# FanmingL/Recurrent-Offpolicy-RL

Hardware: AMD Instinct MI355X
Metric: env-steps/sec trained (higher is better)
Workload: dtype f32; 1 GPU; smamba_s32_c16_b2_nln SAC-REDQ update, B=64/GPU, T=1024, D=256 (configs[1]; N=8: configs[3]); row_length=1043, obs=17, act=6, critic=efc-8, global_rows=64, parallelism=dp1

## Files before the change

recurrent-offpolicy-rl_amd/csrc/gemm_bf3.hip:

```cpp
#include "gemm_splitk.h"
#include "gemm_call.h"

namespace {
using namespace resel;

typedef float f32x16 __attribute__((ext_vector_type(16)));
typedef __bf16 bf16x8 __attribute__((ext_vector_type(8)));
constexpr int BM = 256, BN = 128;
constexpr int NTH = 512;
constexpr int GRID = 256;
constexpr int TILE = BM * BN;
constexpr int ROWB = 64;
constexpr int PLA = BM * ROWB, PLB = BN * ROWB;
constexpr int STAGE = 3 * PLA + 3 * PLB;

struct Params {
    const float *A, *B, *bias;
    float *C, *slab;
    int64_t lda, ldb, ldc, sA, sB, sC, sBias;
    int M, N, K;
    int act;
    int mt, nt;
    int nfull, nsplit, nsl, kslice;
    const float *amaxA, *amaxB;
    AmaxOut amaxC;
    int ntst;
    const float* aux;
    int64_t ldaux, sAux;
    float* red;
    int redrows;
};

__device__ __forceinline__ int plane_off(int row, int c) {
    const int q = row >> 2;
    return ((row ^ (q & 1)) << 6) + ((c ^ (q & 3)) << 4);
}

__device__ __forceinline__ uint32_t rne_pair(float lo, float hi) {
    typedef __bf16 bf16x2_t __attribute__((ext_vector_type(2)));
    typedef float f32x2_t __attribute__((ext_vector_type(2)));
    const f32x2_t v = {lo, hi};
    return __builtin_bit_cast(uint32_t, __builtin_convertvector(v, bf16x2_t));
}
struct P3 { uint2 p1, p2, p3; };
template <int NP>
__device__ __forceinline__ P3 split4(const float4& v) {
#ifdef BF3_AB_NOSPLIT
    return P3{make_uint2(__float_as_uint(v.x), __float_as_uint(v.y)), make_uint2(__float_as_uint(v.z), __float_as_uint(v.w)),
              make_uint2(__float_as_uint(v.x), __float_as_uint(v.w))};
#endif
    const float x[4] = {v.x, v.y, v.z, v.w};
    uint32_t w1[2], w2[2], w3[2] = {0u, 0u};
#pragma unroll
    for (int q = 0; q < 2; ++q) {
        const uint32_t u0 = __float_as_uint(x[2 * q]), u1 = __float_as_uint(x[2 * q + 1]);
        w1[q] = __builtin_amdgcn_perm(u1, u0, 0x07060302u);
        const float r0 = x[2 * q] - __uint_as_float(u0 & 0xffff0000u), r1 = x[2 * q + 1] - __uint_as_float(u1 & 0xffff0000u);
        if (NP == 2) {
            w2[q] = rne_pair(r0, r1);
        } else {
            const uint32_t v0 = __float_as_uint(r0), v1 = __float_as_uint(r1);
            w2[q] = __builtin_amdgcn_perm(v1, v0, 0x07060302u);
            const float s0 = r0 - __uint_as_float(v0 & 0xffff0000u), s1 = r1 - __uint_as_float(v1 & 0xffff0000u);
            w3[q] = __builtin_amdgcn_perm(__float_as_uint(s1), __float_as_uint(s0), 0x07060302u);
        }
    }
    return P3{make_uint2(w1[0], w1[1]), make_uint2(w2[0], w2[1]), make_uint2(w3[0], w3[1])};
}
struct P3h { uint32_t p1, p2, p3; };
template <int NP>
__device__ __forceinline__ P3h split2(float x0, float x1) {
    const uint32_t u0 = __float_as_uint(x0), u1 = __float_as_uint(x1);
    P3h o;
    o.p1 = __builtin_amdgcn_perm(u1, u0, 0x07060302u);
    const float r0 = x0 - __uint_as_float(u0 & 0xffff0000u), r1 = x1 - __uint_as_float(u1 & 0xffff0000u);
    if (NP == 2) {
        o.p2 = rne_pair(r0, r1);
        o.p3 = 0u;
        return o;
    }
    const uint32_t v0 = __float_as_uint(r0), v1 = __float_as_uint(r1);
    o.p2 = __builtin_amdgcn_perm(v1, v0, 0x07060302u);
    const float s0 = r0 - __uint_as_float(v0 & 0xffff0000u), s1 = r1 - __uint_as_float(v1 & 0xffff0000u);
    o.p3 = __builtin_amdgcn_perm(__float_as_uint(s1), __float_as_uint(s0), 0x07060302u);
    return o;
}

typedef _Float16 f16x2_t __attribute__((ext_vector_type(2)));
typedef float f32x2_t __attribute__((ext_vector_type(2)));
template <bool WIDE>
__device__ __forceinline__ void split_pair_f16(float x0, float x1, f32x2_t sc, uint32_t& p1, uint32_t& p2, uint32_t& p3) {
#ifdef BF3_AB_NOSPLIT
    p1 = __float_as_uint(x0); p2 = __float_as_uint(x1); p3 = __float_as_uint(x0) ^ __float_as_uint(sc.x);
    return;
#endif
    const f32x2_t xs = {x0 * sc.x, x1 * sc.x};
    const f16x2_t h = __builtin_convertvector(xs, f16x2_t);
    p1 = __builtin_bit_cast(uint32_t, h);
    if (WIDE) {
        const f32x2_t r = {__builtin_fmaf((float)h.x, -2048.f, x0 * sc.y), __builtin_fmaf((float)h.y, -2048.f, x1 * sc.y)};
        p2 = __builtin_bit_cast(uint32_t, __builtin_convertvector(r, f16x2_t));
        p3 = 0u;
    } else {
        const f32x2_t r = {xs.x - (float)h.x, xs.y - (float)h.y};
        p2 = __builtin_bit_cast(uint32_t, __builtin_convertvector(r, f16x2_t));
        p3 = 0u;
    }
}
template <bool WIDE>
__device__ __forceinline__ P3 split4_f16(const float4& v, f32x2_t sc) {
    P3 o;
    split_pair_f16<WIDE>(v.x, v.y, sc, o.p1.x, o.p2.x, o.p3.x);
    split_pair_f16<WIDE>(v.z, v.w, sc, o.p1.y, o.p2.y, o.p3.y);
// ... 379 lines not shown
            }
            BF3_FENCE();
            cur_st ^= 1;
        }
        if (F16) {
#pragma unroll
            for (int a = 0; a < 2; ++a)
#pragma unroll
                for (int b = 0; b < 2; ++b)
#pragma unroll
                    for (int e = 0; e < 16; ++e) acc[a][b][e] *= unscale;
        }
#ifdef BF3_AB_NOEPI
        if (lane == 0) p.C[(int64_t)cur.m0 * p.ldc + cur.n0 + w] = acc[0][0][0] + acc[0][1][1] + acc[1][0][2] + acc[1][1][3];
        continue;
#endif
        if (cur.split) {
            slab_store<BN>(p.slab + (int64_t)(cur.split - 1) * TILE + (wm + 4 * lh) * BN + wn + li, acc);
        } else {
            float* C = p.C + (int64_t)cur.z * p.sC;
            const bool full_m = cur.m0 + BM <= p.M;
#pragma unroll
            for (int b = 0; b < 2; ++b) {
                const int n = cur.n0 + wn + 32 * b + li;
                if (n >= p.N) continue;
#pragma unroll
                for (int a = 0; a < 2; ++a) {
                    float v[16];
#pragma unroll
                    for (int e = 0; e < 16; ++e) v[e] = acc[a][b][e] + bv[b];
                    if (p.act == 1) {
#pragma unroll
                        for (int e = 0; e < 16; ++e) v[e] = elu1(v[e]);
                    }
                    if (p.act == 3) {
#pragma unroll
                        for (int e = 0; e < 16; ++e) v[e] = softplus_nb(v[e]);
                    }
                    const int mb = cur.m0 + wm + 32 * a + 4 * lh;
                    float* crow = C + (int64_t)mb * p.ldc + n;
                    if (p.act == 2) {
#pragma unroll
                        for (int e = 0; e < 16; ++e) {
                            const int dm = (e & 3) + 8 * (e >> 2);
                            if (mb + dm < p.M) v[e] += crow[(int64_t)dm * p.ldc];
                        }
                    }
                    if (full_m) {
#pragma unroll
                        for (int e = 0; e < 16; ++e) crow[(int64_t)((e & 3) + 8 * (e >> 2)) * p.ldc] = v[e];
                    } else {
#pragma unroll
                        for (int e = 0; e < 16; ++e) {
                            const int dm = (e & 3) + 8 * (e >> 2);
                            if (mb + dm < p.M) crow[(int64_t)dm * p.ldc] = v[e];
                        }
                    }
                    if (p.amaxC.slot) {
#pragma unroll
                        for (int e = 0; e < 16; e += 2) cmax = fmaxf(cmax, fmaxf(__builtin_fabsf(v[e]), __builtin_fabsf(v[e + 1])));
                    }
                }
            }
        }
    }
    amax_publish_wave(cmax, p.amaxC);
#ifdef BF3_AB_CLOCK
    if (tid == 0) {
        g_bf3_clock[2 * blockIdx.x] = __builtin_amdgcn_s_memtime() - ck_t0;
        g_bf3_clock[2 * blockIdx.x + 1] = __builtin_amdgcn_s_memrealtime() - ck_r0;
    }
#endif
}

constexpr int NTH_WS = 512;
constexpr int WS_LDS = 2 * STAGE;
#define WS_BARRIER() asm volatile("s_waitcnt lgkmcnt(0)\n\ts_barrier" ::: "memory")

template <bool AKC, bool BKC, int EPI = 0>
__global__ __launch_bounds__(NTH_WS, 1) void gemm_ws_kernel(Params p) {
    static_assert(EPI == 0 || EPI == 4 || EPI == 5, "EPI: 0 plain, 4 dact, 5 head (the act codes of the fused host entries)");
    extern __shared__ __attribute__((aligned(16))) char lds[];
    const int tid = threadIdx.x;
    const int total = p.nfull + p.nsplit * p.nsl;
    const int G = gridDim.x;
    if ((int)blockIdx.x >= total) return;
    const float sa_ = f16_scale(amax_read(p.amaxA)), sb_ = f16_scale(amax_read(p.amaxB));
    asm volatile("" :: "v"(sa_), "v"(sb_));

    if (__builtin_amdgcn_readfirstlane(tid) >= 256) {
        const int pt = tid - 256;
        const f32x2_t scA = {sa_, 2048.f * sa_}, scB = {sb_, 2048.f * sb_};
        typedef Src<AKC, BM> SA;
        typedef Src<BKC, BN> SB;
        SA a0, a1;
        SB b0, b1;
        a0.init_lds(pt); a1.init_lds(pt + 256);
        b0.init_lds(pt); b1.init_lds(pt + 256);
        typedef float f32x4a __attribute__((ext_vector_type(4)));
        f32x4a ra[2][2][SA::NR], rb[2][2][SB::NR];
        int nsteps = 0;
        for (int it = blockIdx.x; it < total; it += G) {
            const Item i = decode<BM, BN>(p, it);
            nsteps += (i.kend - i.kbeg + BK - 1) / BK;
        }
        int p_item = blockIdx.x, p_k0 = 0, p_kend = 0;
        bool p_live = true;
        auto p_open = [&]() {
            const Item it = decode<BM, BN>(p, p_item);
            const float* Ab = p.A + (int64_t)it.z * p.sA;
            const float* Bb = p.B + (int64_t)it.z * p.sB;
            a0.init(Ab, p.lda, p.M, it.m0, it.kbeg, pt); a1.init(Ab, p.lda, p.M, it.m0, it.kbeg, pt + 256);
            b0.init(Bb, p.ldb, p.N, it.n0, it.kbeg, pt); b1.init(Bb, p.ldb, p.N, it.n0, it.kbeg, pt + 256);
            p_k0 = it.kbeg; p_kend = it.kend;
        };
        auto advance = [&]() {
            a0.base += a0.step; a1.base += a1.step; b0.base += b0.step; b1.base += b1.step;
            p_k0 += BK;
            if (p_k0 >= p_kend) {
                p_item += G;
                if (p_item < total) p_open(); else p_live = false;
            }
        };
        auto aload = [&](f32x4a& r, const char* base, uint32_t off) {
#ifdef BF3_AB_NOLOAD
            asm volatile("" : "+v"(r) : "v"(off), "s"(base) : "memory");
#else
            asm volatile("global_load_dwordx4 %0, %1, %2" : "=v"(r) : "v"(off), "s"(base) : "memory");
#endif
        };
        auto issue_set = [&](auto SET) {
            constexpr int S = decltype(SET)::value;
            auto all = [&](auto& src, auto& regs) {
                typedef std::remove_reference_t<decltype(src)> ST;
#pragma unroll
                for (int i = 0; i < ST::NR; ++i) {
                    if constexpr (ST::is_kc) aload(regs[i], src.base, src.piece_off(i));
                    else aload(regs[i], src.base, src.off[i]);
                }
            };
            all(a0, ra[S][0]); all(a1, ra[S][1]); all(b0, rb[S][0]); all(b1, rb[S][1]);
            advance();
        };
        auto recycle = [&](auto SET, auto MODEC) {
            constexpr int S = decltype(SET)::value;
            constexpr int MODE = decltype(MODEC)::value;
            constexpr bool LOAD = MODE == 0;
            uint32_t st_off = S * STAGE;
            asm volatile("" : "+s"(st_off));
            char* st = lds + st_off;
            auto one = [&](auto& src, auto& regs, char* pl, f32x2_t sc, auto PLc, auto WIDEc) {
                constexpr int PL = decltype(PLc)::value;
                constexpr bool WIDE = decltype(WIDEc)::value;
                typedef std::remove_reference_t<decltype(src)> ST;
                if constexpr (ST::is_kc) {
#pragma unroll
                    for (int i = 0; i < ST::NR; ++i) {
                        if (LOAD) asm volatile("s_waitcnt vmcnt(23)" : "+v"(regs[i]) :: "memory");
                        const float4 v = make_float4(regs[i].x, regs[i].y, regs[i].z, regs[i].w);
                        const P3 sp = split4_f16<WIDE>(v, sc);
                        char* d = pl + src.loff[0] + 4096 * i;
                        *reinterpret_cast<uint2*>(d) = sp.p1;
                        *reinterpret_cast<uint2*>(d + PL) = sp.p2;
                        if (MODE != 1) aload(regs[i], src.base, src.piece_off(i));
                    }
                } else {
                    float4 t[ST::NR];
                    if constexpr (ST::NR == 4) { if (LOAD) asm volatile("s_waitcnt vmcnt(20)" : "+v"(regs[0]), "+v"(regs[1]), "+v"(regs[2]), "+v"(regs[3]) :: "memory"); }
                    else { if (LOAD) asm volatile("s_waitcnt vmcnt(22)" : "+v"(regs[0]), "+v"(regs[1]) :: "memory"); }
#pragma unroll
                    for (int i = 0; i < ST::NR; ++i) t[i] = make_float4(regs[i].x, regs[i].y, regs[i].z, regs[i].w);
                    src.template store_from<PL, 2, WIDE ? 1 : 2>(t, pl, sc);
                    if (MODE != 1) {
#pragma unroll
                        for (int i = 0; i < ST::NR; ++i) aload(regs[i], src.base, src.off[i]);
                    }
                }
            };
            using IA = std::integral_constant<int, PLA>;
            using IB = std::integral_constant<int, PLB>;
            one(a0, ra[S][0], st, scA, IA{}, std::true_type{});
            one(a1, ra[S][1], st, scA, IA{}, std::true_type{});
            one(b0, rb[S][0], st + 3 * PLA, scB, IB{}, std::false_type{});
            one(b1, rb[S][1], st + 3 * PLA, scB, IB{}, std::false_type{});
            if (MODE != 1) advance();
        };
        auto landed = [&]() {
#pragma unroll
            for (int q = 0; q < 2; ++q)
#pragma unroll
                for (int v = 0; v < 2; ++v) {
#pragma unroll
                    for (int i = 0; i < SA::NR; ++i) asm volatile("s_waitcnt vmcnt(0)" : "+v"(ra[q][v][i]) :: "memory");
#pragma unroll
                    for (int i = 0; i < SB::NR; ++i) asm volatile("s_waitcnt vmcnt(0)" : "+v"(rb[q][v][i]) :: "memory");
                }
        };
        using S0 = std::integral_constant<int, 0>;
        using S1 = std::integral_constant<int, 1>;
        using M0 = std::integral_constant<int, 0>;
        using M1 = std::integral_constant<int, 1>;
        using M2 = std::integral_constant<int, 2>;
        p_open();
        issue_set(S0{});
        if (nsteps > 1) issue_set(S1{});
        int j = 0;
        for (; j + 3 < nsteps; j += 2) {
            recycle(S0{}, M0{});
            WS_BARRIER();
            recycle(S1{}, M0{});
            WS_BARRIER();
        }
        landed();
        for (; j < nsteps; ++j) {
            const bool more = j + 2 < nsteps;
            if (j & 1) { if (more) recycle(S1{}, M2{}); else recycle(S1{}, M1{}); }
            else { if (more) recycle(S0{}, M2{}); else recycle(S0{}, M1{}); }
            if (more) landed();
            WS_BARRIER();
        }
        WS_BARRIER();
        return;
    }

    const float unscale = (1.f / sa_) * (1.f / sb_);
    const int lane = tid & 63, w = tid >> 6;
    const int wm = (w >> 1) * 128, wn = (w & 1) * 64;
    const int li = lane & 31, lh = lane >> 5;
    const char* fa[2];
    const char* fb[2];
#pragma unroll
    for (int s = 0; s < 2; ++s) {
        fa[s] = lds + wm * ROWB + plane_off(li, 2 * s + lh);
        fb[s] = lds + 3 * PLA + wn * ROWB + plane_off(li, 2 * s + lh);
    }
    struct F4 { f16x8 a[2][4], b[2][2]; };
    auto rd = [&](F4& f, const char* pa, const char* pb) {
#pragma unroll
        for (int pi = 0; pi < 2; ++pi) {
#pragma unroll
            for (int t = 0; t < 4; ++t) f.a[pi][t] = *reinterpret_cast<const f16x8*>(pa + pi * PLA + t * 32 * ROWB);
#pragma unroll
            for (int t = 0; t < 2; ++t) f.b[pi][t] = *reinterpret_cast<const f16x8*>(pb + pi * PLB + t * 32 * ROWB);
        }
    };
    f32x16 acc[4][2];
    auto mm = [&](const F4& f) {
        const f16x8 k = {(_Float16)0.00048828125f, (_Float16)0.00048828125f, (_Float16)0.00048828125f, (_Float16)0.00048828125f,
                         (_Float16)0.00048828125f, (_Float16)0.00048828125f, (_Float16)0.00048828125f, (_Float16)0.00048828125f};
        const f16x8 bs0 = f.b[0][0] * k, bs1 = f.b[0][1] * k;
#ifdef BF3_AB_NOMFMA
#pragma unroll
        for (int a = 0; a < 4; ++a) asm volatile("" :: "v"(f.a[0][a]), "v"(f.a[1][a]), "v"(bs0), "v"(bs1), "v"(f.b[0][0]), "v"(f.b[0][1]), "v"(f.b[1][0]), "v"(f.b[1][1]));
        return;
#endif
#pragma unroll
        for (int a = 0; a < 4; ++a) {
            acc[a][0] = __builtin_amdgcn_mfma_f32_32x32x16_f16(f.a[1][a], bs0, acc[a][0], 0, 0, 0);
            acc[a][1] = __builtin_amdgcn_mfma_f32_32x32x16_f16(f.a[1][a], bs1, acc[a][1], 0, 0, 0);
        }
#pragma unroll
        for (int q = 1; q >= 0; --q)
#pragma unroll
            for (int a = 0; a < 4; ++a) {
                acc[a][0] = __builtin_amdgcn_mfma_f32_32x32x16_f16(f.a[0][a], f.b[q][0], acc[a][0], 0, 0, 0);
                acc[a][1] = __builtin_amdgcn_mfma_f32_32x32x16_f16(f.a[0][a], f.b[q][1], acc[a][1], 0, 0, 0);
            }
    };
    float cmax = 0.f;
    F4 f0, f1;
    WS_BARRIER();
    rd(f0, fa[0], fb[0]);
    int cur_st = 0;
    constexpr bool DEFER_F0 = EPI == 4;
    for (int c_item = blockIdx.x; c_item < total; c_item += G) {
        const Item cur = decode<BM, BN>(p, c_item);
        if (DEFER_F0 && c_item != (int)blockIdx.x) rd(f0, fa[0] + cur_st * STAGE, fb[0] + cur_st * STAGE);
        float zero = 0.f;
        asm volatile("" : "+v"(zero));
#pragma unroll
        for (int a = 0; a < 4; ++a)
#pragma unroll
            for (int b = 0; b < 2; ++b)
#pragma unroll
                for (int e = 0; e < 16; ++e) acc[a][b][e] = zero;
        float bv[2] = {0.f, 0.f};
        for (int c_k0 = cur.kbeg; c_k0 < cur.kend; c_k0 += BK) {
            const int so = cur_st * STAGE, sn = (cur_st ^ 1) * STAGE;
            if (c_k0 + BK >= cur.kend && p.bias && !cur.split) {
#pragma unroll
                for (int b = 0; b < 2; ++b) {
                    const int n = cur.n0 + wn + 32 * b + li;
                    bv[b] = p.bias[(int64_t)cur.z * p.sBias + (n < p.N ? n : 0)];
                }
            }
            BF3_FENCE();
            rd(f1, fa[1] + so, fb[1] + so);
            mm(f0);
#pragma unroll
            for (int i = 0; i < 12; ++i) {
                __builtin_amdgcn_sched_group_barrier(0x008, 1, 0);
                __builtin_amdgcn_sched_group_barrier(0x100, 1, 0);
            }
            BF3_FENCE();
            WS_BARRIER();
            BF3_FENCE();
            if (!(DEFER_F0 && c_k0 + BK >= cur.kend)) rd(f0, fa[0] + sn, fb[0] + sn);
            mm(f1);
#pragma unroll
            for (int i = 0; i < 12; ++i) {
                __builtin_amdgcn_sched_group_barrier(0x008, 1, 0);
                __builtin_amdgcn_sched_group_barrier(0x100, 1, 0);
            }
            BF3_FENCE();
            cur_st ^= 1;
        }
#ifdef BF3_AB_NOEPI
        if (lane == 0) p.C[(int64_t)cur.m0 * p.ldc + cur.n0 + w] = acc[0][0][0] + acc[1][1][1] + acc[2][0][2] + acc[3][1][3];
        continue;
#endif
#pragma unroll
        for (int a = 0; a < 4; ++a)
#pragma unroll
            for (int b = 0; b < 2; ++b)
#pragma unroll
                for (int e = 0; e < 16; ++e) acc[a][b][e] *= unscale;
        if (cur.split) {
            float* o = p.slab + (int64_t)(cur.split - 1) * TILE + (wm + 4 * lh) * BN + wn + li;
#pragma unroll
            for (int a = 0; a < 4; ++a)
#pragma unroll
                for (int b = 0; b < 2; ++b)
#pragma unroll
                    for (int e = 0; e < 16; ++e) o[(32 * a + (e & 3) + 8 * (e >> 2)) * BN + 32 * b] = acc[a][b][e];
            continue;
        }
        if constexpr (EPI == 0) {
            float* C = p.C + (int64_t)cur.z * p.sC;
            const bool full_m = cur.m0 + BM <= p.M;
            if (full_m && cur.n0 + BN <= p.N && p.act != 2) {
                char* sc = lds + (w >> 1) * STAGE + 2 * PLA + (w & 1) * 5120;
                float* wr = reinterpret_cast<float*>(sc) + (4 * lh) * 40 + li;
                const float4* rdp = reinterpret_cast<const float4*>(sc + (lane >> 3) * 160 + (lane & 7) * 16);
#pragma unroll
                for (int b = 0; b < 2; ++b) {
#pragma unroll
                    for (int a = 0; a < 4; ++a) {
                        float v[16];
#pragma unroll
                        for (int e = 0; e < 16; ++e) v[e] = acc[a][b][e] + bv[b];
                        if (p.act == 1) {
#pragma unroll
                            for (int e = 0; e < 16; ++e) v[e] = elu1(v[e]);
                        }
                        if (p.act == 3) {
#pragma unroll
                            for (int e = 0; e < 16; ++e) v[e] = softplus_nb(v[e]);
                        }
                        if (p.amaxC.slot) {
#pragma unroll
                            for (int e = 0; e < 16; e += 2) cmax = fmaxf(cmax, fmaxf(__builtin_fabsf(v[e]), __builtin_fabsf(v[e + 1])));
                        }
#pragma unroll
                        for (int e = 0; e < 16; ++e) wr[((e & 3) + 8 * (e >> 2)) * 40] = v[e];
                        float* q = C + (int64_t)(cur.m0 + wm + 32 * a + (lane >> 3)) * p.ldc + cur.n0 + wn + 32 * b + 4 * (lane & 7);
#pragma unroll
                        for (int g = 0; g < 4; ++g) {
                            const float4 t = rdp[g * 8 * 10];
                            if (p.ntst) {
                                typedef float f4v __attribute__((ext_vector_type(4)));
                                __builtin_nontemporal_store(f4v{t.x, t.y, t.z, t.w}, reinterpret_cast<f4v*>(q + (int64_t)(8 * g) * p.ldc));
                            } else {
                                *reinterpret_cast<float4*>(q + (int64_t)(8 * g) * p.ldc) = t;
                            }
                        }
                    }
                }
                continue;
            }
#pragma unroll
            for (int b = 0; b < 2; ++b) {
                const int n = cur.n0 + wn + 32 * b + li;
                if (n >= p.N) continue;
#pragma unroll
                for (int a = 0; a < 4; ++a) {
                    float v[16];
#pragma unroll
                    for (int e = 0; e < 16; ++e) v[e] = acc[a][b][e] + bv[b];
                    if (p.act == 1) {
#pragma unroll
                        for (int e = 0; e < 16; ++e) v[e] = elu1(v[e]);
                    }
                    if (p.act == 3) {
#pragma unroll
                        for (int e = 0; e < 16; ++e) v[e] = softplus_nb(v[e]);
                    }
                    const int mb = cur.m0 + wm + 32 * a + 4 * lh;
                    float* crow = C + (int64_t)mb * p.ldc + n;
                    if (p.act == 2) {
#pragma unroll
                        for (int e = 0; e < 16; ++e) {
                            const int dm = (e & 3) + 8 * (e >> 2);
                            if (mb + dm < p.M) v[e] += crow[(int64_t)dm * p.ldc];
                        }
                    }
                    if (full_m) {
#pragma unroll
                        for (int e = 0; e < 16; ++e) crow[(int64_t)((e & 3) + 8 * (e >> 2)) * p.ldc] = v[e];
                    } else {
#pragma unroll
                        for (int e = 0; e < 16; ++e) {
                            const int dm = (e & 3) + 8 * (e >> 2);
                            if (mb + dm < p.M) crow[(int64_t)dm * p.ldc] = v[e];
                        }
                    }
                    if (p.amaxC.slot) {
#pragma unroll
                        for (int e = 0; e < 16; e += 2) cmax = fmaxf(cmax, fmaxf(__builtin_fabsf(v[e]), __builtin_fabsf(v[e + 1])));
                    }
                }
            }
        } else if constexpr (EPI == 4) {
            float* C = p.C + (int64_t)cur.z * p.sC;
            constexpr int PF = 3;
            const int lane = (int)__builtin_amdgcn_mbcnt_hi(~0u, __builtin_amdgcn_mbcnt_lo(~0u, 0u));
            const int li = lane & 31, lh = lane >> 5;
            const int w = __builtin_amdgcn_readfirstlane(threadIdx.x >> 6);
            const int wm = (w >> 1) * 128, wn = (w & 1) * 64;
            typedef float f32x4a __attribute__((ext_vector_type(4)));
            f32x4a yv[8][4];
            char* sc = lds + (w >> 1) * STAGE + 2 * PLA + (w & 1) * 5120;
            float* wr = reinterpret_cast<float*>(sc) + (4 * lh) * 40 + li;
            float4* rdp = reinterpret_cast<float4*>(sc + (lane >> 3) * 160 + (lane & 7) * 16);
            const uint32_t ylane = (uint32_t)(((lane >> 3) * (int)p.ldaux + 4 * (lane & 7)) * 4);
            const float* ybase = p.aux + (int64_t)cur.z * p.sAux + (int64_t)(cur.m0 + wm) * p.ldaux + cur.n0 + wn;
            auto yld = [](f32x4a& r, uint32_t off, const float* base) {
                asm volatile("global_load_dwordx4 %0, %1, %2" : "=v"(r) : "v"(off), "s"(base) : "memory");
            };
            auto ywait = [](f32x4a& r0, f32x4a& r1, f32x4a& r2, f32x4a& r3, auto NC) {
                asm volatile("s_waitcnt vmcnt(%4)" : "+v"(r0), "+v"(r1), "+v"(r2), "+v"(r3) : "n"(decltype(NC)::value) : "memory");
            };
            auto yload = [&](auto TC) {
                constexpr int t = decltype(TC)::value;
                if constexpr (t < 8) {
                    const float* yb = ybase + (int64_t)(32 * (t >> 1)) * p.ldaux + 32 * (t & 1);
#pragma unroll
                    for (int g = 0; g < 4; ++g) yld(yv[t][g], ylane, yb + (int64_t)(8 * g) * p.ldaux);
                }
            };
            float cs[2] = {0.f, 0.f}, cmx = 0.f;
            auto mul = [&](auto TC) {
                constexpr int t = decltype(TC)::value;
                constexpr int a = t >> 1, b = t & 1;
                yload(std::integral_constant<int, t + PF>{});
                ywait(yv[t][0], yv[t][1], yv[t][2], yv[t][3], std::integral_constant<int, 4 * ((t + PF < 7 ? t + PF : 7) - t)>{});
#pragma unroll
                for (int g = 0; g < 4; ++g) rdp[g * 8 * 10] = make_float4(yv[t][g].x, yv[t][g].y, yv[t][g].z, yv[t][g].w);
#pragma unroll
                for (int e = 0; e < 16; ++e) {
                    const float y = wr[((e & 3) + 8 * (e >> 2)) * 40];
                    const float v = acc[a][b][e] * (y > 0.f ? 1.f : y + 1.f);
                    acc[a][b][e] = v;
                    cs[b] += v;
                    cmx = fmaxf(cmx, __builtin_fabsf(v));
                }
            };
            yload(std::integral_constant<int, 0>{}); yload(std::integral_constant<int, 1>{}); yload(std::integral_constant<int, 2>{});
            static_assert(PF == 3, "the prologue issues PF tiles");
            mul(std::integral_constant<int, 0>{}); mul(std::integral_constant<int, 1>{}); mul(std::integral_constant<int, 2>{});
            mul(std::integral_constant<int, 3>{}); mul(std::integral_constant<int, 4>{}); mul(std::integral_constant<int, 5>{});
            mul(std::integral_constant<int, 6>{}); mul(std::integral_constant<int, 7>{});
            if (p.red) {
#pragma unroll
                for (int b = 0; b < 2; ++b) {
                    const float c = cs[b] + __shfl_xor(cs[b], 32, 64);
                    if (lh == 0) p.red[((int64_t)cur.z * p.redrows + 2 * (cur.m0 / BM) + (w >> 1)) * p.N + cur.n0 + wn + 32 * b + li] = c;
                }
            }
            amax_publish_wave(cmx, p.amaxC);
#pragma unroll
            for (int b = 0; b < 2; ++b) {
#pragma unroll
                for (int a = 0; a < 4; ++a) {
#pragma unroll
                    for (int e = 0; e < 16; ++e) wr[((e & 3) + 8 * (e >> 2)) * 40] = acc[a][b][e];
                    float* q = C + (int64_t)(cur.m0 + wm + 32 * a + (lane >> 3)) * p.ldc + cur.n0 + wn + 32 * b + 4 * (lane & 7);
#pragma unroll
                    for (int g = 0; g < 4; ++g) {
                        const float4 t = rdp[g * 8 * 10];
                        typedef float f4v __attribute__((ext_vector_type(4)));
                        __builtin_nontemporal_store(f4v{t.x, t.y, t.z, t.w}, reinterpret_cast<f4v*>(q + (int64_t)(8 * g) * p.ldc));
                    }
                }
            }
        } else {
            float* C = p.C + (int64_t)cur.z * p.sC;
            const bool full_m = cur.m0 + BM <= p.M;
            if (full_m && cur.n0 + BN <= p.N) {
                char* sc = lds + (w >> 1) * STAGE + 2 * PLA + (w & 1) * 5120;
                float* wr = reinterpret_cast<float*>(sc) + (4 * lh) * 40 + li;
                const float4* rdp = reinterpret_cast<const float4*>(sc + (lane >> 3) * 160 + (lane & 7) * 16);
                auto tile = [&](int a, int b, const float4& w3, float (&qr)[4]) {
                    float v[16];
#pragma unroll
                    for (int e = 0; e < 16; ++e) v[e] = acc[a][b][e] + bv[b];
#pragma unroll
                    for (int e = 0; e < 16; ++e) v[e] = elu1(v[e]);
                    if (p.amaxC.slot) {
#pragma unroll
                        for (int e = 0; e < 16; e += 2) cmax = fmaxf(cmax, fmaxf(__builtin_fabsf(v[e]), __builtin_fabsf(v[e + 1])));
                    }
#pragma unroll
                    for (int e = 0; e < 16; ++e) wr[((e & 3) + 8 * (e >> 2)) * 40] = v[e];
                    float* q = C + (int64_t)(cur.m0 + wm + 32 * a + (lane >> 3)) * p.ldc + cur.n0 + wn + 32 * b + 4 * (lane & 7);
#pragma unroll
                    for (int g = 0; g < 4; ++g) {
                        float4 t = rdp[g * 8 * 10];
                        qr[g] += (t.x * w3.x + t.y * w3.y) + (t.z * w3.z + t.w * w3.w);
                        if (p.ntst) {
                            typedef float f4v __attribute__((ext_vector_type(4)));
                            __builtin_nontemporal_store(f4v{t.x, t.y, t.z, t.w}, reinterpret_cast<f4v*>(q + (int64_t)(8 * g) * p.ldc));
                        } else {
                            *reinterpret_cast<float4*>(q + (int64_t)(8 * g) * p.ldc) = t;
                        }
                    }
                };
                float4 w3[2];
#pragma unroll
                for (int b = 0; b < 2; ++b) w3[b] = ld4(p.aux + (int64_t)cur.z * p.sAux + cur.n0 + wn + 32 * b + 4 * (lane & 7));
#pragma unroll
                for (int a = 0; a < 4; ++a) {
                    float qr[4] = {0.f, 0.f, 0.f, 0.f};
#pragma unroll
                    for (int b = 0; b < 2; ++b) tile(a, b, w3[b], qr);
                    float* qp = p.red + ((int64_t)cur.z * 2 * p.nt + 2 * (cur.n0 / BN) + (w & 1)) * p.M + cur.m0 + wm + 32 * a + (lane >> 3);
#pragma unroll
                    for (int g = 0; g < 4; ++g) {
                        float r = qr[g];
                        r += __shfl_xor(r, 1, 64); r += __shfl_xor(r, 2, 64); r += __shfl_xor(r, 4, 64);
                        if ((lane & 7) == 0) qp[8 * g] = r;
                    }
                }
                continue;
            }
#pragma unroll
            for (int a = 0; a < 4; ++a) {
                float qe[16];
#pragma unroll
                for (int e = 0; e < 16; ++e) qe[e] = 0.f;
                const int mb = cur.m0 + wm + 32 * a + 4 * lh;
#pragma unroll
                for (int b = 0; b < 2; ++b) {
                    const int n = cur.n0 + wn + 32 * b + li;
                    if (n >= p.N) continue;
                    float v[16];
#pragma unroll
                    for (int e = 0; e < 16; ++e) v[e] = acc[a][b][e] + bv[b];
#pragma unroll
                    for (int e = 0; e < 16; ++e) v[e] = elu1(v[e]);
                    const float w3 = p.aux[(int64_t)cur.z * p.sAux + n];
#pragma unroll
                    for (int e = 0; e < 16; ++e) qe[e] += v[e] * w3;
                    float* crow = C + (int64_t)mb * p.ldc + n;
                    if (full_m) {
#pragma unroll
                        for (int e = 0; e < 16; ++e) crow[(int64_t)((e & 3) + 8 * (e >> 2)) * p.ldc] = v[e];
                    } else {
#pragma unroll
                        for (int e = 0; e < 16; ++e) {
                            const int dm = (e & 3) + 8 * (e >> 2);
                            if (mb + dm < p.M) crow[(int64_t)dm * p.ldc] = v[e];
                        }
                    }
                    if (p.amaxC.slot) {
#pragma unroll
                        for (int e = 0; e < 16; e += 2) cmax = fmaxf(cmax, fmaxf(__builtin_fabsf(v[e]), __builtin_fabsf(v[e + 1])));
                    }
                }
                float* qp = p.red + ((int64_t)cur.z * 2 * p.nt + 2 * (cur.n0 / BN) + (w & 1)) * p.M;
#pragma unroll
                for (int e = 0; e < 16; ++e) {
                    float r = qe[e];
#pragma unroll
                    for (int o = 1; o < 32; o <<= 1) r += __shfl_xor(r, o, 64);
                    const int m = mb + (e & 3) + 8 * (e >> 2);
                    if (li == 0 && m < p.M) qp[m] = r;
                }
            }
        }
    }
    amax_publish_wave(cmax, p.amaxC);
}

template <bool AKC, bool BKC, int SP>
int launch_one(const Params& p, dim3 grid, hipStream_t s) {
    static std::atomic<bool> attr_set[64];
    return launch_big_lds(gemm_bf3_kernel<AKC, BKC, SP>, attr_set, grid, dim3(NTH), 2 * STAGE, s, p);
}
template <bool AKC, bool BKC, int EPI = 0>
int launch_ws(const Params& p, dim3 grid, hipStream_t s) {
    static std::atomic<bool> attr_set[64];
    return launch_big_lds(gemm_ws_kernel<AKC, BKC, EPI>, attr_set, grid, dim3(NTH_WS), WS_LDS, s, p);
}

constexpr int g_nt = 1;

}

#ifdef BF3_AB_CLOCK
extern "C" int resel_bf3_debug_clock(unsigned long long* host_out) {
    return (int)hipMemcpyFromSymbol(host_out, HIP_SYMBOL(g_bf3_clock), sizeof(unsigned long long) * 2 * GRID);
}
#endif

namespace resel {

size_t gemm_bf3_workspace_bytes(int M, int N, int K, int batch) {
    const Plan pl = make_plan<BM, BN, GRID>(M, N, K, batch);
    return (size_t)pl.nsplit * pl.nsl * TILE * sizeof(float);
}

inline bool whole_k_steps(int K, int kslice) { return K % BK == 0 && kslice % BK == 0; }

bool gemm_bf3_fused_ok(int M, int N, int K) { return M > 128 && N >= 4 && K >= BK && whole_k_steps(K, K); }

int gemm_bf3_launch(const GemmCall& c, int split, const GemmFused& fused) {
    if (split == 2 && (!c.amax_a || !c.amax_b)) return RESEL_EINVAL;
    const int M = c.M, N = c.N, K = c.K, act = c.act;
    Plan pl = make_plan<BM, BN, GRID>(M, N, K, c.batch);
    if (act >= 4) {
        if (split != 2 || !gemm_bf3_fused_ok(M, N, K) || !fused.aux) return RESEL_EINVAL;
        if (act == 4 && (M % BM || N % BN)) return RESEL_EINVAL;
        if (!c.a_kcontig) return RESEL_EINVAL;
        const long nbt = (long)((M + BM - 1) / BM) * ((N + BN - 1) / BN) * c.batch;
        pl = Plan{(int)nbt, 0, 1, (K + BK - 1) / BK * BK};
    }
    if (pl.nsplit && (!c.workspace || !aligned16(c.workspace))) return RESEL_EINVAL;
    Params p{(const float*)c.A, c.B, c.bias, (float*)c.C, (float*)c.workspace, c.lda, c.ldb, c.ldc, c.strideA, c.strideB, c.strideC, c.strideBias,
             M, N, K, act, (M + BM - 1) / BM, (N + BN - 1) / BN, pl.nfull, pl.nsplit, pl.nsl, pl.kslice, c.amax_a, c.amax_b,
             AmaxOut{c.amax_c, c.amax_epoch}, g_nt, fused.aux, fused.ldaux, fused.strideAux, fused.red, fused.redrows};
    dim3 grid((unsigned)std::min<int64_t>((int64_t)pl.nfull + (int64_t)pl.nsplit * pl.nsl, GRID));
    const bool third = split == 2 && whole_k_steps(K, pl.kslice);
    const int rc = with_layout(c.a_kcontig, c.b_kcontig, [&](auto akc, auto bkc) {
        constexpr bool AKC = akc.value, BKC = bkc.value;
        if constexpr (AKC) {
            if (act >= 4) return act == 4 ? launch_ws<true, BKC, 4>(p, grid, c.s) : launch_ws<true, BKC, 5>(p, grid, c.s);
        }
        if (third) return launch_ws<AKC, BKC>(p, grid, c.s);
        if (split == 3) return launch_one<AKC, BKC, 3>(p, grid, c.s);
        if (split == 2) return launch_one<AKC, BKC, 2>(p, grid, c.s);
        return launch_one<AKC, BKC, 6>(p, grid, c.s);
    });
    if (rc != RESEL_OK) return rc;
    if (pl.nsplit) hipLaunchKernelGGL((gemm_fixup_kernel<BM, BN, Params>), dim3(TILE / 4 / 64, pl.nsplit), dim3(64, 4), 0, c.s, p);
#ifdef BF3_AB_FIXUP2
    if (pl.nsplit && act != 2) hipLaunchKernelGGL((gemm_fixup_kernel<BM, BN, Params>), dim3(TILE / 4 / 64, pl.nsplit), dim3(64, 4), 0, c.s, p);
#endif
    return launch_status();
}

}
```

recurrent-offpolicy-rl_amd/csrc/gemm_splitk.h:

```cpp
#pragma once
#include "resel_common.h"
#include <algorithm>
#include <atomic>

namespace resel {

constexpr int BK = 32;

__device__ __forceinline__ float elu1(float x) { return x > 0.f ? x : fast_exp(x) - 1.f; }

template <int BN, typename ACC, int NA>
__device__ __forceinline__ void slab_store(float* o, const ACC (&acc)[NA][2]) {
#pragma unroll
    for (int a = 0; a < NA; ++a)
#pragma unroll
        for (int b = 0; b < 2; ++b)
#pragma unroll
            for (int e = 0; e < 16; ++e) o[(32 * a + (e & 3) + 8 * (e >> 2)) * BN + 32 * b] = acc[a][b][e];
}

template <int BM, int BN, typename P>
__device__ __forceinline__ void tile_origin(const P& p, int t, int& z, int& m0, int& n0) {
    const int ntile = p.mt * p.nt;
    z = t / ntile;
    const int tt = t - z * ntile;
    const int q = ntile / 8, r = ntile % 8, x = tt & 7, j = tt >> 3;
    const int bid = (x < r ? x * (q + 1) : r * (q + 1) + (x - r) * q) + j;
    m0 = (bid / p.nt) * BM;
    n0 = (bid % p.nt) * BN;
}

struct Item { int m0, n0, z, kbeg, kend, split; };
template <int BM, int BN, typename P>
__device__ __forceinline__ Item decode(const P& p, int it) {
    Item o;
    int t = it;
    o.kbeg = 0; o.kend = p.K; o.split = 0;
    if (it >= p.nfull) {
        const int idx = it - p.nfull, tr = idx / p.nsl, sl = idx - tr * p.nsl;
        t = p.nfull + tr;
        o.kbeg = sl * p.kslice; o.kend = min(p.K, o.kbeg + p.kslice); o.split = idx + 1;
    }
    tile_origin<BM, BN>(p, t, o.z, o.m0, o.n0);
    return o;
}

template <int BM, int BN, typename P>
__global__ __launch_bounds__(256) void gemm_fixup_kernel(P p) {
    static_assert(BN == 128, "a slab row is 32 float4");
    constexpr int TILE = BM * BN;
    __shared__ float4 part[3][64];
    const int tr = blockIdx.y, q = threadIdx.y;
    const int e = blockIdx.x * 64 + threadIdx.x, ml = e >> 5, nl = 4 * (e & 31);
    const float* s = p.slab + (int64_t)tr * p.nsl * TILE + ml * BN + nl;
    float4 v = make_float4(0.f, 0.f, 0.f, 0.f);
    int i = q;
    for (; i + 12 < p.nsl; i += 16) {
        const float4 u0 = ld4(s + (int64_t)i * TILE), u1 = ld4(s + (int64_t)(i + 4) * TILE);
        const float4 u2 = ld4(s + (int64_t)(i + 8) * TILE), u3 = ld4(s + (int64_t)(i + 12) * TILE);
        v.x = (((v.x + u0.x) + u1.x) + u2.x) + u3.x; v.y = (((v.y + u0.y) + u1.y) + u2.y) + u3.y;
        v.z = (((v.z + u0.z) + u1.z) + u2.z) + u3.z; v.w = (((v.w + u0.w) + u1.w) + u2.w) + u3.w;
    }
    for (; i < p.nsl; i += 4) {
        const float4 u = ld4(s + (int64_t)i * TILE);
        v.x += u.x; v.y += u.y; v.z += u.z; v.w += u.w;
    }
    if (q) part[q - 1][threadIdx.x] = v;
    __syncthreads();
    if (q) return;
    const float4 g1 = part[0][threadIdx.x], g2 = part[1][threadIdx.x], g3 = part[2][threadIdx.x];
    float o[4] = {(v.x + g1.x) + (g2.x + g3.x), (v.y + g1.y) + (g2.y + g3.y), (v.z + g1.z) + (g2.z + g3.z), (v.w + g1.w) + (g2.w + g3.w)};
    int z, m0, n0;
    tile_origin<BM, BN>(p, p.nfull + tr, z, m0, n0);
    const int m = m0 + ml, n = n0 + nl;
    float cmax = 0.f;
    if (m < p.M && n < p.N) {
        float* c = p.C + (int64_t)z * p.sC + (int64_t)m * p.ldc + n;
#pragma unroll
        for (int j = 0; j < 4; ++j) {
            if (n + j >= p.N) break;
            float x = o[j] + (p.bias ? p.bias[(int64_t)z * p.sBias + n + j] : 0.f);
            if (p.act == 1) x = elu1(x);
            if (p.act == 3) x = softplus_nb(x);
            if (p.act == 2) x += c[j];
            c[j] = x;
            cmax = fmaxf(cmax, __builtin_fabsf(x));
        }
    }
    amax_publish_wave(cmax, p.amaxC);
}

struct Plan { int nfull, nsplit, nsl, kslice; };
constexpr int g_split_min_ksteps = 4;
template <int BM, int BN, int GRID>
inline Plan make_plan(int M, int N, int K, int batch) {
    const long nbt = (long)((M + BM - 1) / BM) * ((N + BN - 1) / BN) * batch;
    const int ksteps = (K + BK - 1) / BK;
    Plan pl{(int)nbt, 0, 1, ksteps * BK};
    const int r = (int)(nbt % GRID);
    if (r == 0 || r > GRID / 2 || ksteps < g_split_min_ksteps) return pl;
    int s = std::min(GRID / r, ksteps / 2);
    const int per = (ksteps + s - 1) / s;
    s = (ksteps + per - 1) / per;
    if (s < 2) return pl;
    pl.nfull = (int)(nbt - r); pl.nsplit = r; pl.nsl = s; pl.kslice = per * BK;
    return pl;
}

template <typename K, typename P>
inline int launch_big_lds(K kernel, std::atomic<bool> (&attr_set)[64], dim3 grid, dim3 block, int lds, hipStream_t s, const P& p) {
    int dev = 0;
    if (hipGetDevice(&dev) != hipSuccess || dev < 0 || dev >= 64) return RESEL_ELAUNCH;
    if (!attr_set[dev].load(std::memory_order_acquire)) {
        if (hipFuncSetAttribute((const void*)kernel, hipFuncAttributeMaxDynamicSharedMemorySize, lds) != hipSuccess) return RESEL_ELAUNCH;
        attr_set[dev].store(true, std::memory_order_release);
    }
    launch_timed(RESEL_PROF_GEMM, kernel, grid, block, (size_t)lds, s, p);
    return RESEL_OK;
}

}
```

Before: 3.011 million env-steps/s.

## Add row-piece tail splitting to GEMM planner as alternative to split-K

Adds a new way to spread the leftover tail tiles of a persistent GEMM across idle blocks: each tail tile is split into row pieces that each run the full K loop, with no slab writes or fixup pass. A simple cost model in make_plan picks between split-K and row splitting. The producer skips converting A rows it does not own, the consumer runs a reduced MFMA loop with masked epilogues, and the head-fused path can now be split too. This removes the split-K reduction traffic and fixup launch for tail tiles, at the price of reloading B per piece and more complex control flow.

```diff
diff --git a/recurrent-offpolicy-rl_amd/csrc/gemm_bf3.hip b/recurrent-offpolicy-rl_amd/csrc/gemm_bf3.hip
--- a/recurrent-offpolicy-rl_amd/csrc/gemm_bf3.hip
+++ b/recurrent-offpolicy-rl_amd/csrc/gemm_bf3.hip
@@ -29,6 +29,7 @@
     int64_t ldaux, sAux;
     float* red;
     int redrows;
+    int nrow, npc, prows;
 };
 
 __device__ __forceinline__ int plane_off(int row, int c) {
@@ -574,7 +575,7 @@
     static_assert(EPI == 0 || EPI == 4 || EPI == 5, "EPI: 0 plain, 4 dact, 5 head (the act codes of the fused host entries)");
     extern __shared__ __attribute__((aligned(16))) char lds[];
     const int tid = threadIdx.x;
-    const int total = p.nfull + p.nsplit * p.nsl;
+    const int total = p.nfull + p.nsplit * p.nsl + p.nrow * p.npc;
     const int G = gridDim.x;
     if ((int)blockIdx.x >= total) return;
     const float sa_ = f16_scale(amax_read(p.amaxA)), sb_ = f16_scale(amax_read(p.amaxB));
@@ -591,18 +592,19 @@
         b0.init_lds(pt); b1.init_lds(pt + 256);
         typedef float f32x4a __attribute__((ext_vector_type(4)));
         f32x4a ra[2][2][SA::NR], rb[2][2][SB::NR];
-        int nsteps = 0;
+        int nsteps = 0, nwhole = 0, pblk = BM / 32;
         for (int it = blockIdx.x; it < total; it += G) {
-            const Item i = decode<BM, BN>(p, it);
+            const Item i = decode_rows<BM, BN>(p, it);
             nsteps += (i.kend - i.kbeg + BK - 1) / BK;
+            if (i.rows == BM) nwhole = nsteps; else pblk = i.rows >> 5;
         }
         int p_item = blockIdx.x, p_k0 = 0, p_kend = 0;
         bool p_live = true;
         auto p_open = [&]() {
-            const Item it = decode<BM, BN>(p, p_item);
+            const Item it = decode_rows<BM, BN>(p, p_item);
             const float* Ab = p.A + (int64_t)it.z * p.sA;
             const float* Bb = p.B + (int64_t)it.z * p.sB;
-            a0.init(Ab, p.lda, p.M, it.m0, it.kbeg, pt); a1.init(Ab, p.lda, p.M, it.m0, it.kbeg, pt + 256);
+            a0.init(Ab, p.lda, it.mlim, it.m0, it.kbeg, pt); a1.init(Ab, p.lda, it.mlim, it.m0, it.kbeg, pt + 256);
             b0.init(Bb, p.ldb, p.N, it.n0, it.kbeg, pt); b1.init(Bb, p.ldb, p.N, it.n0, it.kbeg, pt + 256);
             p_k0 = it.kbeg; p_kend = it.kend;
         };
@@ -634,14 +636,14 @@
             all(a0, ra[S][0]); all(a1, ra[S][1]); all(b0, rb[S][0]); all(b1, rb[S][1]);
             advance();
         };
-        auto recycle = [&](auto SET, auto MODEC) {
+        auto recycle = [&](auto SET, auto MODEC, auto own) {
             constexpr int S = decltype(SET)::value;
             constexpr int MODE = decltype(MODEC)::value;
             constexpr bool LOAD = MODE == 0;
             uint32_t st_off = S * STAGE;
             asm volatile("" : "+s"(st_off));
             char* st = lds + st_off;
-            auto one = [&](auto& src, auto& regs, char* pl, f32x2_t sc, auto PLc, auto WIDEc) {
+            auto one = [&](auto& src, auto& regs, char* pl, f32x2_t sc, auto PLc, auto WIDEc, int vt) {
                 constexpr int PL = decltype(PLc)::value;
                 constexpr bool WIDE = decltype(WIDEc)::value;
                 typedef std::remove_reference_t<decltype(src)> ST;
@@ -649,11 +651,13 @@
 #pragma unroll
                     for (int i = 0; i < ST::NR; ++i) {
                         if (LOAD) asm volatile("s_waitcnt vmcnt(23)" : "+v"(regs[i]) :: "memory");
-                        const float4 v = make_float4(regs[i].x, regs[i].y, regs[i].z, regs[i].w);
-                        const P3 sp = split4_f16<WIDE>(v, sc);
-                        char* d = pl + src.loff[0] + 4096 * i;
-                        *reinterpret_cast<uint2*>(d) = sp.p1;
-                        *reinterpret_cast<uint2*>(d + PL) = sp.p2;
+                        if (!WIDE || 2 * i + vt < own) {
+                            const float4 v = make_float4(regs[i].x, regs[i].y, regs[i].z, regs[i].w);
+                            const P3 sp = split4_f16<WIDE>(v, sc);
+                            char* d = pl + src.loff[0] + 4096 * i;
+                            *reinterpret_cast<uint2*>(d) = sp.p1;
+                            *reinterpret_cast<uint2*>(d + PL) = sp.p2;
+                        }
                         if (MODE != 1) aload(regs[i], src.base, src.piece_off(i));
                     }
                 } else {
@@ -671,10 +675,10 @@
             };
             using IA = std::integral_constant<int, PLA>;
             using IB = std::integral_constant<int, PLB>;
-            one(a0, ra[S][0], st, scA, IA{}, std::true_type{});
-            one(a1, ra[S][1], st, scA, IA{}, std::true_type{});
-            one(b0, rb[S][0], st + 3 * PLA, scB, IB{}, std::false_type{});
-            one(b1, rb[S][1], st + 3 * PLA, scB, IB{}, std::false_type{});
+            one(a0, ra[S][0], st, scA, IA{}, std::true_type{}, 0);
+            one(a1, ra[S][1], st, scA, IA{}, std::true_type{}, 1);
+            one(b0, rb[S][0], st + 3 * PLA, scB, IB{}, std::false_type{}, 0);
+            one(b1, rb[S][1], st + 3 * PLA, scB, IB{}, std::false_type{}, 1);
             if (MODE != 1) advance();
         };
         auto landed = [&]() {
@@ -698,16 +702,26 @@
         if (nsteps > 1) issue_set(S1{});
         int j = 0;
         for (; j + 3 < nsteps; j += 2) {
-            recycle(S0{}, M0{});
+            if (SA::is_kc && j + 1 >= nwhole) break;
+            recycle(S0{}, M0{}, std::integral_constant<int, BM / 32>{});
             WS_BARRIER();
-            recycle(S1{}, M0{});
+            recycle(S1{}, M0{}, std::integral_constant<int, BM / 32>{});
             WS_BARRIER();
+        }
+        if constexpr (SA::is_kc) {
+            for (; j + 3 < nsteps; j += 2) {
+                recycle(S0{}, M0{}, j < nwhole ? BM / 32 : pblk);
+                WS_BARRIER();
+                recycle(S1{}, M0{}, j + 1 < nwhole ? BM / 32 : pblk);
+                WS_BARRIER();
+            }
         }
         landed();
         for (; j < nsteps; ++j) {
             const bool more = j + 2 < nsteps;
-            if (j & 1) { if (more) recycle(S1{}, M2{}); else recycle(S1{}, M1{}); }
-            else { if (more) recycle(S0{}, M2{}); else recycle(S0{}, M1{}); }
+            const int own = j < nwhole ? BM / 32 : pblk;
+            if (j & 1) { if (more) recycle(S1{}, M2{}, own); else recycle(S1{}, M1{}, own); }
+            else { if (more) recycle(S0{}, M2{}, own); else recycle(S0{}, M1{}, own); }
             if (more) landed();
             WS_BARRIER();
         }
@@ -758,6 +772,22 @@
                 acc[a][0] = __builtin_amdgcn_mfma_f32_32x32x16_f16(f.a[0][a], f.b[q][0], acc[a][0], 0, 0, 0);
                 acc[a][1] = __builtin_amdgcn_mfma_f32_32x32x16_f16(f.a[0][a], f.b[q][1], acc[a][1], 0, 0, 0);
             }
+    };
+    auto mm_rows = [&](const F4& f, int na) {
+        const f16x8 k = {(_Float16)0.00048828125f, (_Float16)0.00048828125f, (_Float16)0.00048828125f, (_Float16)0.00048828125f,
+                         (_Float16)0.00048828125f, (_Float16)0.00048828125f, (_Float16)0.00048828125f, (_Float16)0.00048828125f};
+        const f16x8 bs0 = f.b[0][0] * k, bs1 = f.b[0][1] * k;
+#pragma unroll
+        for (int a = 0; a < 4; ++a) {
+            if (a >= na) break;
+            acc[a][0] = __builtin_amdgcn_mfma_f32_32x32x16_f16(f.a[1][a], bs0, acc[a][0], 0, 0, 0);
+            acc[a][1] = __builtin_amdgcn_mfma_f32_32x32x16_f16(f.a[1][a], bs1, acc[a][1], 0, 0, 0);
+#pragma unroll
+            for (int q = 1; q >= 0; --q) {
+                acc[a][0] = __builtin_amdgcn_mfma_f32_32x32x16_f16(f.a[0][a], f.b[q][0], acc[a][0], 0, 0, 0);
+                acc[a][1] = __builtin_amdgcn_mfma_f32_32x32x16_f16(f.a[0][a], f.b[q][1], acc[a][1], 0, 0, 0);
+            }
+        }
     };
     float cmax = 0.f;
     F4 f0, f1;
@@ -766,7 +796,8 @@
     int cur_st = 0;
     constexpr bool DEFER_F0 = EPI == 4;
     for (int c_item = blockIdx.x; c_item < total; c_item += G) {
-        const Item cur = decode<BM, BN>(p, c_item);
+        const Item cur = decode_rows<BM, BN>(p, c_item);
+        const int wrows = __builtin_amdgcn_readfirstlane(cur.rows - wm);
         if (DEFER_F0 && c_item != (int)blockIdx.x) rd(f0, fa[0] + cur_st * STAGE, fb[0] + cur_st * STAGE);
         float zero = 0.f;
         asm volatile("" : "+v"(zero));
@@ -777,7 +808,27 @@
 #pragma unroll
                 for (int e = 0; e < 16; ++e) acc[a][b][e] = zero;
         float bv[2] = {0.f, 0.f};
-        for (int c_k0 = cur.kbeg; c_k0 < cur.kend; c_k0 += BK) {
+        const bool piece = EPI != 4 && cur.rows < BM;
+        if (piece) {
+            const int na = min(max(wrows >> 5, 0), 4);
+            for (int c_k0 = 0; c_k0 < cur.kend; c_k0 += BK) {
+                const int so = cur_st * STAGE, sn = (cur_st ^ 1) * STAGE;
+                if (c_k0 + BK >= cur.kend && p.bias) {
+#pragma unroll
+                    for (int b = 0; b < 2; ++b) {
+                        const int n = cur.n0 + wn + 32 * b + li;
+                        bv[b] = p.bias[(int64_t)cur.z * p.sBias + (n < p.N ? n : 0)];
+                    }
+                }
+                rd(f1, fa[1] + so, fb[1] + so);
+                mm_rows(f0, na);
+                WS_BARRIER();
+                rd(f0, fa[0] + sn, fb[0] + sn);
+                mm_rows(f1, na);
+                cur_st ^= 1;
+            }
+        }
+        for (int c_k0 = cur.kbeg; c_k0 < cur.kend && !piece; c_k0 += BK) {
             const int so = cur_st * STAGE, sn = (cur_st ^ 1) * STAGE;
             if (c_k0 + BK >= cur.kend && p.bias && !cur.split) {
 #pragma unroll
@@ -829,7 +880,7 @@
         }
         if constexpr (EPI == 0) {
             float* C = p.C + (int64_t)cur.z * p.sC;
-            const bool full_m = cur.m0 + BM <= p.M;
+            const bool full_m = !piece && cur.m0 + BM <= p.M;
             if (full_m && cur.n0 + BN <= p.N && p.act != 2) {
                 char* sc = lds + (w >> 1) * STAGE + 2 * PLA + (w & 1) * 5120;
                 float* wr = reinterpret_cast<float*>(sc) + (4 * lh) * 40 + li;
@@ -870,12 +921,47 @@
                 }
                 continue;
             }
+            if (piece && cur.m0 + cur.rows <= p.M && cur.n0 + BN <= p.N && p.act != 2) {
+                char* sc = lds + (w >> 1) * STAGE + 2 * PLA + (w & 1) * 5120;
+                float* wr = reinterpret_cast<float*>(sc) + (4 * lh) * 40 + li;
+                const float4* rdp = reinterpret_cast<const float4*>(sc + (lane >> 3) * 160 + (lane & 7) * 16);
+#pragma unroll
+                for (int a = 0; a < 4; ++a) {
+                    if (32 * a >= wrows) break;
+#pragma unroll
+                    for (int b = 0; b < 2; ++b) {
+                        float v[16];
+#pragma unroll
+                        for (int e = 0; e < 16; ++e) v[e] = acc[a][b][e] + bv[b];
+                        if (p.act == 1) {
+#pragma unroll
+                            for (int e = 0; e < 16; ++e) v[e] = elu1(v[e]);
+                        }
+                        if (p.act == 3) {
+#pragma unroll
+                            for (int e = 0; e < 16; ++e) v[e] = softplus_nb(v[e]);
+                        }
+                        if (p.amaxC.slot) {
+#pragma unroll
+                            for (int e = 0; e < 16; e += 2) cmax = fmaxf(cmax, fmaxf(__builtin_fabsf(v[e]), __builtin_fabsf(v[e + 1])));
+                        }
+#pragma unroll
+                        for (int e = 0; e < 16; ++e) wr[((e & 3) + 8 * (e >> 2)) * 40] = v[e];
+                        float* q = C + (int64_t)(cur.m0 + wm + 32 * a + (lane >> 3)) * p.ldc + cur.n0 + wn + 32 * b + 4 * (lane & 7);
+#pragma unroll
+                        for (int g = 0; g < 4; ++g) *reinterpret_cast<float4*>(q + (int64_t)(8 * g) * p.ldc) = rdp[g * 8 * 10];
+                    }
+                }
+                continue;
+            }
+            const bool all_m = full_m && cur.rows == BM;
 #pragma unroll
             for (int b = 0; b < 2; ++b) {
                 const int n = cur.n0 + wn + 32 * b + li;
                 if (n >= p.N) continue;
 #pragma unroll
                 for (int a = 0; a < 4; ++a) {
+                    if (32 * a >= wrows) break;
                     float v[16];
 #pragma unroll
                     for (int e = 0; e < 16; ++e) v[e] = acc[a][b][e] + bv[b];
@@ -893,17 +979,17 @@
 #pragma unroll
                         for (int e = 0; e < 16; ++e) {
                             const int dm = (e & 3) + 8 * (e >> 2);
-                            if (mb + dm < p.M) v[e] += crow[(int64_t)dm * p.ldc];
-                        }
-                    }
-                    if (full_m) {
+                            if (mb + dm < cur.mlim) v[e] += crow[(int64_t)dm * p.ldc];
+                        }
+                    }
+                    if (all_m) {
 #pragma unroll
                         for (int e = 0; e < 16; ++e) crow[(int64_t)((e & 3) + 8 * (e >> 2)) * p.ldc] = v[e];
                     } else {
 #pragma unroll
                         for (int e = 0; e < 16; ++e) {
                             const int dm = (e & 3) + 8 * (e >> 2);
-                            if (mb + dm < p.M) crow[(int64_t)dm * p.ldc] = v[e];
+                            if (mb + dm < cur.mlim) crow[(int64_t)dm * p.ldc] = v[e];
                         }
                     }
                     if (p.amaxC.slot) {
@@ -987,7 +1073,7 @@
             }
         } else {
             float* C = p.C + (int64_t)cur.z * p.sC;
-            const bool full_m = cur.m0 + BM <= p.M;
+            const bool full_m = cur.m0 + cur.rows <= p.M;
             if (full_m && cur.n0 + BN <= p.N) {
                 char* sc = lds + (w >> 1) * STAGE + 2 * PLA + (w & 1) * 5120;
                 float* wr = reinterpret_cast<float*>(sc) + (4 * lh) * 40 + li;
@@ -1022,6 +1108,7 @@
                 for (int b = 0; b < 2; ++b) w3[b] = ld4(p.aux + (int64_t)cur.z * p.sAux + cur.n0 + wn + 32 * b + 4 * (lane & 7));
 #pragma unroll
                 for (int a = 0; a < 4; ++a) {
+                    if (32 * a >= wrows) break;
                     float qr[4] = {0.f, 0.f, 0.f, 0.f};
 #pragma unroll
                     for (int b = 0; b < 2; ++b) tile(a, b, w3[b], qr);
@@ -1037,6 +1124,7 @@
             }
 #pragma unroll
             for (int a = 0; a < 4; ++a) {
+                if (32 * a >= wrows) break;
                 float qe[16];
 #pragma unroll
                 for (int e = 0; e < 16; ++e) qe[e] = 0.f;
@@ -1054,14 +1142,14 @@
 #pragma unroll
                     for (int e = 0; e < 16; ++e) qe[e] += v[e] * w3;
                     float* crow = C + (int64_t)mb * p.ldc + n;
-                    if (full_m) {
+                    if (full_m && cur.rows == BM) {
 #pragma unroll
                         for (int e = 0; e < 16; ++e) crow[(int64_t)((e & 3) + 8 * (e >> 2)) * p.ldc] = v[e];
                     } else {
 #pragma unroll
                         for (int e = 0; e < 16; ++e) {
                             const int dm = (e & 3) + 8 * (e >> 2);
-                            if (mb + dm < p.M) crow[(int64_t)dm * p.ldc] = v[e];
+                            if (mb + dm < cur.mlim) crow[(int64_t)dm * p.ldc] = v[e];
                         }
                     }
                     if (p.amaxC.slot) {
@@ -1076,7 +1164,7 @@
 #pragma unroll
                     for (int o = 1; o < 32; o <<= 1) r += __shfl_xor(r, o, 64);
                     const int m = mb + (e & 3) + 8 * (e >> 2);
-                    if (li == 0 && m < p.M) qp[m] = r;
+                    if (li == 0 && m < cur.mlim) qp[m] = r;
                 }
             }
         }
@@ -1107,6 +1195,8 @@
 
 namespace resel {
 
+int g_row_cut = [] { const char* e = getenv("RESEL_GEMM_ROW_CUT"); return e ? atoi(e) : 1; }();
+
 size_t gemm_bf3_workspace_bytes(int M, int N, int K, int batch) {
     const Plan pl = make_plan<BM, BN, GRID>(M, N, K, batch);
     return (size_t)pl.nsplit * pl.nsl * TILE * sizeof(float);
@@ -1119,19 +1209,19 @@
 int gemm_bf3_launch(const GemmCall& c, int split, const GemmFused& fused) {
     if (split == 2 && (!c.amax_a || !c.amax_b)) return RESEL_EINVAL;
     const int M = c.M, N = c.N, K = c.K, act = c.act;
-    Plan pl = make_plan<BM, BN, GRID>(M, N, K, c.batch);
+    const int rows_cut = split == 2 && K % BK == 0 && c.a_kcontig && g_row_cut ? CUT_ROWS : 0;
+    Plan pl = make_plan<BM, BN, GRID>(M, N, K, c.batch, CUT_K | rows_cut, g_row_cut == 2);
     if (act >= 4) {
         if (split != 2 || !gemm_bf3_fused_ok(M, N, K) || !fused.aux) return RESEL_EINVAL;
         if (act == 4 && (M % BM || N % BN)) return RESEL_EINVAL;
         if (!c.a_kcontig) return RESEL_EINVAL;
-        const long nbt = (long)((M + BM - 1) / BM) * ((N + BN - 1) / BN) * c.batch;
-        pl = Plan{(int)nbt, 0, 1, (K + BK - 1) / BK * BK};
+        pl = make_plan<BM, BN, GRID>(M, N, K, c.batch, act == 5 ? rows_cut : 0, g_row_cut == 2);
     }
     if (pl.nsplit && (!c.workspace || !aligned16(c.workspace))) return RESEL_EINVAL;
     Params p{(const float*)c.A, c.B, c.bias, (float*)c.C, (float*)c.workspace, c.lda, c.ldb, c.ldc, c.strideA, c.strideB, c.strideC, c.strideBias,
              M, N, K, act, (M + BM - 1) / BM, (N + BN - 1) / BN, pl.nfull, pl.nsplit, pl.nsl, pl.kslice, c.amax_a, c.amax_b,
-             AmaxOut{c.amax_c, c.amax_epoch}, g_nt, fused.aux, fused.ldaux, fused.strideAux, fused.red, fused.redrows};
-    dim3 grid((unsigned)std::min<int64_t>((int64_t)pl.nfull + (int64_t)pl.nsplit * pl.nsl, GRID));
+             AmaxOut{c.amax_c, c.amax_epoch}, g_nt, fused.aux, fused.ldaux, fused.strideAux, fused.red, fused.redrows, pl.nrow, pl.npc, pl.prows};
+    dim3 grid((unsigned)std::min<int64_t>((int64_t)pl.nfull + (int64_t)pl.nsplit * pl.nsl + (int64_t)pl.nrow * pl.npc, GRID));
     const bool third = split == 2 && whole_k_steps(K, pl.kslice);
     const int rc = with_layout(c.a_kcontig, c.b_kcontig, [&](auto akc, auto bkc) {
         constexpr bool AKC = akc.value, BKC = bkc.value;
diff --git a/recurrent-offpolicy-rl_amd/csrc/gemm_splitk.h b/recurrent-offpolicy-rl_amd/csrc/gemm_splitk.h
--- a/recurrent-offpolicy-rl_amd/csrc/gemm_splitk.h
+++ b/recurrent-offpolicy-rl_amd/csrc/gemm_splitk.h
@@ -30,7 +30,10 @@
     n0 = (bid % p.nt) * BN;
 }
 
-struct Item { int m0, n0, z, kbeg, kend, split; };
+struct Item {
+    int m0, n0, z, kbeg, kend, split;
+    int rows, mlim;
+};
 template <int BM, int BN, typename P>
 __device__ __forceinline__ Item decode(const P& p, int it) {
     Item o;
@@ -42,6 +45,22 @@
         o.kbeg = sl * p.kslice; o.kend = min(p.K, o.kbeg + p.kslice); o.split = idx + 1;
     }
     tile_origin<BM, BN>(p, t, o.z, o.m0, o.n0);
+    o.rows = BM; o.mlim = p.M;
+    return o;
+}
+template <int BM, int BN, typename P>
+__device__ __forceinline__ Item decode_rows(const P& p, int it) {
+    if (!p.nrow || it < p.nfull) return decode<BM, BN>(p, it);
+    Item o;
+    const int idx = it - p.nfull, tr = idx / p.npc, pc = idx - tr * p.npc;
+    o.kbeg = 0; o.kend = p.K; o.split = 0;
+    tile_origin<BM, BN>(p, p.nfull + tr, o.z, o.m0, o.n0);
+    const int mp = o.m0 + pc * p.prows;
+    if (mp < p.M) {
+        o.m0 = mp; o.rows = min(p.prows, BM - pc * p.prows); o.mlim = min(p.M, mp + o.rows);
+    } else {
+        o.rows = 0; o.mlim = o.m0 + 1;
+    }
     return o;
 }
 
@@ -90,20 +109,35 @@
     amax_publish_wave(cmax, p.amaxC);
 }
 
-struct Plan { int nfull, nsplit, nsl, kslice; };
+constexpr int CUT_K = 1, CUT_ROWS = 2;
+struct Plan { int nfull, nsplit, nsl, kslice; int nrow = 0, npc = 1, prows = 0; };
 constexpr int g_split_min_ksteps = 4;
+constexpr float COST_STORE = 4.f, COST_BSHARE = 1.f / 3.f, COST_FIXUP = 3.f, COST_SLABS = 3.f, COST_PIECE_STEP = 0.65f;
 template <int BM, int BN, int GRID>
-inline Plan make_plan(int M, int N, int K, int batch) {
+inline Plan make_plan(int M, int N, int K, int batch, int cuts = CUT_K, bool rows_always = false) {
     const long nbt = (long)((M + BM - 1) / BM) * ((N + BN - 1) / BN) * batch;
     const int ksteps = (K + BK - 1) / BK;
     Plan pl{(int)nbt, 0, 1, ksteps * BK};
     const int r = (int)(nbt % GRID);
-    if (r == 0 || r > GRID / 2 || ksteps < g_split_min_ksteps) return pl;
-    int s = std::min(GRID / r, ksteps / 2);
-    const int per = (ksteps + s - 1) / s;
-    s = (ksteps + per - 1) / per;
-    if (s < 2) return pl;
-    pl.nfull = (int)(nbt - r); pl.nsplit = r; pl.nsl = s; pl.kslice = per * BK;
+    if (r == 0 || r > GRID / 2) return pl;
+    float cost = (float)ksteps + COST_STORE;
+    if ((cuts & CUT_K) && ksteps >= g_split_min_ksteps) {
+        int s = std::min(GRID / r, ksteps / 2);
+        const int per = (ksteps + s - 1) / s;
+        s = (ksteps + per - 1) / per;
+        if (s >= 2) {
+            pl.nfull = (int)(nbt - r); pl.nsplit = r; pl.nsl = s; pl.kslice = per * BK;
+            cost = (float)per + COST_STORE + COST_FIXUP + COST_SLABS * (float)(r * s) / GRID;
+        }
+    }
+    if (!(cuts & CUT_ROWS)) return pl;
+    constexpr int NB = BM / 32;
+    const int pcs = std::min(GRID / r, NB);
+    if (pcs < 2) return pl;
+    const int rb = (NB + pcs - 1) / pcs, npc = (NB + rb - 1) / rb;
+    const float share = (float)rb / NB;
+    const float cost_rows = (float)ksteps * std::max(COST_BSHARE + (1.f - COST_BSHARE) * share, COST_PIECE_STEP) + COST_STORE * share;
+    if (cost_rows < cost || rows_always) pl = Plan{(int)(nbt - r), 0, 1, ksteps * BK, r, npc, 32 * rb};
     return pl;
 }
 
```

New measurement: 3.010 million env-steps/s. Within noise of the previous version (-0.0%).
